# Rayhane-mamah/Tacotron-2

Measured on NVIDIA H100. Metric: wavenet_train_audio_samples_per_sec, higher is better.
Workload: dtype bf16

## Files before the change

### include/t2b200.h

```cpp
#ifndef T2B200_H_
#define T2B200_H_

#include <stdint.h>

#ifdef __cplusplus
extern "C" {
#endif

#define T2B200_ABI_VERSION 2

#define T2_OK 0
#define T2_ERR_INVALID_ARG (-1)
#define T2_ERR_UNSUPPORTED_SHAPE (-2)
#define T2_ERR_CUDA (-3)
#define T2_ERR_NCCL (-4)

const char* t2_last_error(void);
int t2_abi_version(void);
int t2_struct_size(const char* name);
long long t2_launch_count(void);

int t2_dbg_conv_gemm(const void* d_a, int B, int T, int C, int ld, const int* shifts, int nshift,
                     const void* d_w, int N, int BN, const float* d_bias, int relu, void* d_out_bf16,
                     float* d_out_f32, void* stream);
// ... 20 lines not shown
  int cluster_used;
  void* ptr[12];
  float f[6];
  int i[12];
  unsigned long long seed;
} t2_dbg_gemm_t;
int t2_dbg_act_gemm(t2_dbg_gemm_t* call, void* stream);
typedef struct {
  int a_map, a_ch0, a_shift, a_layer;
  int b_map, b_ch0, b_shift, b_layer;
  long long out_off;
  int ldc, m_valid, n_valid;
  float scale;
  int accumulate;
  const float* div;
} t2_dbg_wgrad_tile_t;
int t2_dbg_wgrad_tiles(const t2_dbg_act_t* maps, int nmaps, const t2_dbg_wgrad_tile_t* tiles, int ntiles, float* d_out, int T, int B,
                       void* stream);
int t2_dbg_fx_colsum(const float* d_addends, int nrows, int ncols, float* d_out, void* stream);

typedef struct {
  int kernel;
  void* p[16];
  long long i[16];
  float f[4];
  unsigned long long seed;
  const unsigned long long* step;
} t2_dbg_kernel_t;
#define T2_DBG_TACO_ATT_FWD 1
#define T2_DBG_TACO_BN_FWD 2
// ... 197 lines not shown
```

### tacotron-2_b200/csrc/t2_api.cu

```cuda
#include <stdarg.h>
#include <stdio.h>
#include <stddef.h>
#include <string.h>

#include <vector>

#include "../../include/t2b200.h"
#include "t2_common.cuh"
#include "t2_gemm.h"

#include <atomic>
static thread_local char g_err[512] = "";
static std::atomic<long long> g_launches{0};
void t2_count_launch(int n) { g_launches.fetch_add(n, std::memory_order_relaxed); }
extern "C" long long t2_launch_count(void) { return g_launches.load(std::memory_order_relaxed); }

int t2_set_error(int code, const char* fmt, ...) {
  va_list ap;
  va_start(ap, fmt);
  vsnprintf(g_err, sizeof(g_err), fmt, ap);
  va_end(ap);
  return code;
}

// ... 48 lines not shown
}

#define T2_SAME_FIELD(A, B, f) static_assert(offsetof(A, f) == offsetof(B, f), #A " / " #B ": field " #f)
static_assert(sizeof(t2_dbg_act_t) == sizeof(t2::ActT), "t2_dbg_act_t / ActT");
T2_SAME_FIELD(t2_dbg_act_t, t2::ActT, ptr); T2_SAME_FIELD(t2_dbg_act_t, t2::ActT, C); T2_SAME_FIELD(t2_dbg_act_t, t2::ActT, ld);
static_assert(sizeof(t2_dbg_seg_t) == sizeof(t2::Seg), "t2_dbg_seg_t / Seg");
T2_SAME_FIELD(t2_dbg_seg_t, t2::Seg, map); T2_SAME_FIELD(t2_dbg_seg_t, t2::Seg, nlayers);
static_assert(sizeof(t2_dbg_wgrad_tile_t) == sizeof(t2::WgradTile), "t2_dbg_wgrad_tile_t / WgradTile");
T2_SAME_FIELD(t2_dbg_wgrad_tile_t, t2::WgradTile, a_map); T2_SAME_FIELD(t2_dbg_wgrad_tile_t, t2::WgradTile, a_ch0);
T2_SAME_FIELD(t2_dbg_wgrad_tile_t, t2::WgradTile, a_shift); T2_SAME_FIELD(t2_dbg_wgrad_tile_t, t2::WgradTile, a_layer);
T2_SAME_FIELD(t2_dbg_wgrad_tile_t, t2::WgradTile, b_map); T2_SAME_FIELD(t2_dbg_wgrad_tile_t, t2::WgradTile, b_ch0);
T2_SAME_FIELD(t2_dbg_wgrad_tile_t, t2::WgradTile, b_shift); T2_SAME_FIELD(t2_dbg_wgrad_tile_t, t2::WgradTile, b_layer);
T2_SAME_FIELD(t2_dbg_wgrad_tile_t, t2::WgradTile, out_off); T2_SAME_FIELD(t2_dbg_wgrad_tile_t, t2::WgradTile, ldc);
T2_SAME_FIELD(t2_dbg_wgrad_tile_t, t2::WgradTile, m_valid); T2_SAME_FIELD(t2_dbg_wgrad_tile_t, t2::WgradTile, n_valid);
T2_SAME_FIELD(t2_dbg_wgrad_tile_t, t2::WgradTile, scale); T2_SAME_FIELD(t2_dbg_wgrad_tile_t, t2::WgradTile, accumulate);
T2_SAME_FIELD(t2_dbg_wgrad_tile_t, t2::WgradTile, div);
#undef T2_SAME_FIELD

extern "C" int t2_dbg_act_gemm(t2_dbg_gemm_t* call, void* stream) {
  using namespace t2;
  T2_REQUIRE(call != nullptr, T2_ERR_INVALID_ARG, "null call");
  T2_REQUIRE(call->na >= 1 && call->na <= 4 && call->nseg >= 1 && call->nseg <= kMaxSeg, T2_ERR_INVALID_ARG,
             "bad map/segment count (%d, %d)", call->na, call->nseg);
  ActGemmCall c;
  memset(&c, 0, sizeof(c));
  memcpy(c.a, call->a, sizeof(c.a));
  c.na = call->na;
  memcpy(c.seg, call->seg, sizeof(c.seg));
  c.nseg = call->nseg;
  c.w = call->w; c.wN = call->wN; c.wK = call->wK; c.wL = call->wL; c.w_layer = call->w_layer; c.w_k0 = call->w_k0;
  c.T = call->T; c.B = call->B; c.n_tiles = call->n_tiles; c.ksplit = call->ksplit; c.cluster = call->cluster;
  memcpy(c.epi.ptr, call->ptr, sizeof(c.epi.ptr));
  memcpy(c.epi.f, call->f, sizeof(c.epi.f));
  memcpy(c.epi.i, call->i, sizeof(c.epi.i));
  c.epi.seed = call->seed;
  call->cluster_used = 0;
  return launch_act_gemm(call->epi, call->BN, c, static_cast<cudaStream_t>(stream), &call->cluster_used);
}

extern "C" int t2_dbg_wgrad_tiles(const t2_dbg_act_t* maps, int nmaps, const t2_dbg_wgrad_tile_t* tiles, int ntiles, float* d_out, int T,
                                  int B, void* stream) {
  using namespace t2;
  T2_REQUIRE(maps && tiles && nmaps >= 1 && nmaps <= 6 && ntiles >= 1, T2_ERR_INVALID_ARG, "wgrad_tiles: bad map/tile arguments");
  for (int i = 0; i < ntiles; ++i)
    T2_REQUIRE(tiles[i].a_map >= 0 && tiles[i].a_map < nmaps && tiles[i].b_map >= 0 && tiles[i].b_map < nmaps &&
               tiles[i].m_valid >= 1 && tiles[i].m_valid <= 128 && tiles[i].n_valid >= 1 && tiles[i].n_valid <= 256 &&
               tiles[i].accumulate >= 0 && tiles[i].accumulate <= 2,
               T2_ERR_INVALID_ARG, "wgrad_tiles: bad tile %d", i);
  WgradTile* dt = nullptr;
  cudaStream_t st = static_cast<cudaStream_t>(stream);
  T2_CHECK_CUDA(cudaMallocAsync(&dt, ntiles * sizeof(WgradTile), st));
  const cudaError_t e = cudaMemcpyAsync(dt, tiles, ntiles * sizeof(WgradTile), cudaMemcpyHostToDevice, st);
  int rc = e == cudaSuccess ? launch_wgrad(reinterpret_cast<const ActT*>(maps), nmaps, dt, ntiles, d_out, T, B, st)
                            : t2_set_error(T2_ERR_CUDA, "wgrad_tiles: tile table upload failed: %s", cudaGetErrorString(e));
  cudaStreamSynchronize(st);
  cudaFreeAsync(dt, st);
  return rc;
}

__global__ void fx_colsum_kernel(const float* __restrict__ v, long long n, int ncols, long long* acc) {
  const long long i = blockIdx.x * (long long)blockDim.x + threadIdx.x;
  if (i < n) t2::fx_add(acc + i % ncols, v[i]);
}
extern "C" int t2_dbg_fx_colsum(const float* d_addends, int nrows, int ncols, float* d_out, void* stream) {
  T2_REQUIRE(d_addends && d_out && nrows >= 0 && ncols >= 1, T2_ERR_INVALID_ARG, "fx_colsum: bad arguments");
  cudaStream_t st = static_cast<cudaStream_t>(stream);
  long long* acc = nullptr;
  T2_CHECK_CUDA(cudaMallocAsync(&acc, size_t(ncols) * sizeof(long long), st));
// ... 48 lines not shown
```

### tacotron-2_b200/csrc/t2_gemm.cu

```cuda
#include <stdlib.h>
#include <mutex>

#include "t2_gemm.cuh"
#include "t2_gemm.h"

namespace t2 {

static long long* g_timing_buffer = nullptr;
void set_timing_buffer(long long* p) { g_timing_buffer = p; }

typedef CUresult (*EncodeTiledFn)(CUtensorMap*, CUtensorMapDataType, cuuint32_t, void*, const cuuint64_t*,
                                  const cuuint64_t*, const cuuint32_t*, const cuuint32_t*,
                                  CUtensorMapInterleave, CUtensorMapSwizzle, CUtensorMapL2promotion,
                                  CUtensorMapFloatOOBfill);

static EncodeTiledFn get_encode_fn() {
  static EncodeTiledFn fn = nullptr;
  static std::once_flag once;
  std::call_once(once, [] {
    void* p = nullptr;
    cudaDriverEntryPointQueryResult q;
    if (cudaGetDriverEntryPoint("cuTensorMapEncodeTiled", &p, cudaEnableDefault, &q) == cudaSuccess &&
        q == cudaDriverEntryPointSuccess)
      fn = reinterpret_cast<EncodeTiledFn>(p);
// ... 176 lines not shown
  T2_CASE(EPI_BIAS_ACT, 256)
  T2_CASE(EPI_CE, 256)
  T2_CASE(EPI_SCALE_RELUMASK, 128)
  T2_CASE(EPI_SCALE_RELUMASK, 256)
  T2_CASE(EPI_GATE_BWD, 128)
  T2_CASE(EPI_GATE_BWD, 256)
  T2_CASE(EPI_DX, 128)
  T2_CASE(EPI_DX, 256)
  T2_CASE(EPI_MOL, 32)
  T2_CASE(EPI_LSTM, 32)
  T2_CASE(EPI_TOUT, 32)
#undef T2_CASE
  return t2_set_error(T2_ERR_UNSUPPORTED_SHAPE, "act_gemm: no kernel for epilogue %d with BN=%d", epi, BN);
}

int launch_wgrad(const ActT* maps, int nmaps, const WgradTile* tiles_dev, int ntiles, float* out, int T,
                 int B, cudaStream_t stream) {
  T2_REQUIRE(nmaps >= 1 && nmaps <= 6 && ntiles >= 1, T2_ERR_INVALID_ARG, "wgrad: bad map/tile count");
  WgradArgs g;
  memset(&g, 0, sizeof(g));
  for (int i = 0; i < 6; ++i) {
    int rc = encode_act_map(&g.map[i], maps[i < nmaps ? i : 0], kBK);
    if (rc) return rc;
  }
  g.tiles = tiles_dev;
  g.out = out;
  g.T = T;
  g.B = B;
  static bool configured = false;
  if (!configured) {
    T2_CHECK_CUDA(cudaFuncSetAttribute(wgrad_gemm_kernel, cudaFuncAttributeMaxDynamicSharedMemorySize, kWgSmemBytes));
    configured = true;
  }
  cudaLaunchConfig_t cfg;
  memset(&cfg, 0, sizeof(cfg));
  cfg.gridDim = dim3(ntiles); cfg.blockDim = dim3(kGemmThreads); cfg.dynamicSmemBytes = kWgSmemBytes; cfg.stream = stream;
  cudaLaunchAttribute attr[1];
  attr[0].id = cudaLaunchAttributeProgrammaticStreamSerialization;
  attr[0].val.programmaticStreamSerializationAllowed = 1;
  cfg.attrs = attr; cfg.numAttrs = pdl_enabled() ? 1 : 0;
  T2_CHECK_CUDA(cudaLaunchKernelEx(&cfg, wgrad_gemm_kernel, g));
  t2_count_launch();
  return T2_OK;
}

}
```

### tacotron-2_b200/csrc/t2_gemm.cuh

```cuda
#pragma once
#include "t2_common.cuh"
#include "t2_gemm_types.h"

namespace t2 {

__device__ __forceinline__ void store_bf16x32(__nv_bfloat16* dst, const float (&v)[32]) {
  uint4* d = reinterpret_cast<uint4*>(dst);
#pragma unroll
  for (int q = 0; q < 4; ++q) {
    uint4 u;
    u.x = pack_bf16x2(v[q * 8 + 0], v[q * 8 + 1]);
    u.y = pack_bf16x2(v[q * 8 + 2], v[q * 8 + 3]);
    u.z = pack_bf16x2(v[q * 8 + 4], v[q * 8 + 5]);
    u.w = pack_bf16x2(v[q * 8 + 6], v[q * 8 + 7]);
    d[q] = u;
  }
}
__device__ __forceinline__ void load_bf16x32(const __nv_bfloat16* src, float (&v)[32]) {
  const uint4* s = reinterpret_cast<const uint4*>(src);
#pragma unroll
  for (int q = 0; q < 4; ++q) {
    uint4 u = __ldg(s + q);
    v[q * 8 + 0] = bf16lo(u.x); v[q * 8 + 1] = bf16hi(u.x);
    v[q * 8 + 2] = bf16lo(u.y); v[q * 8 + 3] = bf16hi(u.y);
// ... 984 lines not shown
    asm volatile("bar.sync 6, 512;\n" ::: "memory");
    const int row = q * 32 + lane;
    c.trow = AccRow{acc_s + row * BN, 0, row & 7};
    if (dbg && threadIdx.x == 0) dbg[4] = clock64();
    Epilogue<EPI, BN>::run(g.epi, c);
    if (dbg && threadIdx.x == 0) dbg[5] = clock64();
    tile_store_drain(c);
  }
  __syncthreads();
  if (dbg && threadIdx.x == 0) { dbg[6] = clock64(); dbg[10] = globaltimer_ns(); }
  if (cs > 1) cluster_sync_all();
}

constexpr int kWgBN = 256;
constexpr int kWgStages = 4;
constexpr int kWgStageBytes = 6 * (kBK * 128);
constexpr int kWgSmemBytes = kWgStages * kWgStageBytes + 1024 + 256;
static_assert(kWgSmemBytes <= 232448, "shared memory budget");

template <int N>
__device__ __forceinline__ void wgrad_consume(const WgradArgs& g, const WgradTile& tile, uint8_t* smem, uint64_t* full_bar,
                                              uint64_t* empty_bar, int total_kb) {
  constexpr int kBlk = kBK * 128;
  const int warp = threadIdx.x >> 5, lane = threadIdx.x & 31, wg = warp >> 2;
  float d[N / 2];
#pragma unroll
  for (int i = 0; i < N / 2; ++i) d[i] = 0.f;
  int stage = 0, prev = 0;
  uint32_t phase = 0;
  for (int kb = 0; kb < total_kb; ++kb) {
    mbar_wait(&full_bar[stage], phase);
    __syncwarp();
    const uint32_t sa = smem_u32(smem + stage * kWgStageBytes) + uint32_t(wg * kBlk);
    const uint32_t sb = smem_u32(smem + stage * kWgStageBytes + 2 * kBlk);
    const uint64_t adesc = make_gdesc_sw128(sa, kBlk, 1024);
    const uint64_t bdesc = make_gdesc_sw128(sb, kBlk, 1024);
    wgmma_fence();
    wgmma_fence_regs(d);
#pragma unroll
    for (int k = 0; k < kBK / 16; ++k)
      Wgmma<N, 1, 1>::mma(d, adesc + uint64_t(k * 128), bdesc + uint64_t(k * 128), (kb > 0 || k > 0) ? 1u : 0u);
    wgmma_commit();
    wgmma_fence_regs(d);
    wgmma_wait<1>();
    if (kb > 0 && lane == 0) mbar_arrive(&empty_bar[prev]);
    prev = stage;
    if (++stage == kWgStages) { stage = 0; phase ^= 1; }
  }
  wgmma_wait<0>();
  wgmma_fence_regs(d);
  float sc = tile.scale;
  if (tile.div) sc /= fmaxf(__ldg(tile.div), 1e-20f);
  float* out = g.out + tile.out_off;
  const int m0 = wg * 64 + (warp & 3) * 16 + (lane >> 2);
#pragma unroll
  for (int j = 0; j < N / 8; ++j)
#pragma unroll
    for (int i = 0; i < 2; ++i)
#pragma unroll
      for (int e = 0; e < 2; ++e) {
        const int m = m0 + 8 * i, n = 8 * j + 2 * (lane & 3) + e;
        if (m < tile.m_valid && n < tile.n_valid) {
          float* o = out + size_t(m) * tile.ldc + n;
          const float r = d[4 * j + 2 * i + e] * sc;
          if (tile.accumulate == 2) atomicAdd(o, r);
          else if (tile.accumulate == 1) *o += r;
          else *o = r;
        }
      }
}

__global__ void __launch_bounds__(kGemmThreads, 1) wgrad_gemm_kernel(const __grid_constant__ WgradArgs g) {
  extern __shared__ uint8_t smem_raw[];
  uint8_t* smem = reinterpret_cast<uint8_t*>((reinterpret_cast<uintptr_t>(smem_raw) + 1023) & ~uintptr_t(1023));
  uint64_t* full_bar = reinterpret_cast<uint64_t*>(smem + kWgStages * kWgStageBytes);
  uint64_t* empty_bar = full_bar + kWgStages;
  const int warp = threadIdx.x >> 5;
  const WgradTile tile = g.tiles[blockIdx.x];
  const int kb_per_b = (g.T + kBK - 1) / kBK;
  const int total_kb = kb_per_b * g.B;
  const int nblk = (tile.n_valid + 63) >> 6;

  if (warp == 8 && elect_one()) {
    for (int i = 0; i < kWgStages; ++i) { mbar_init(&full_bar[i], 1); mbar_init(&empty_bar[i], 8); }
    fence_barrier_init();
  }
  __syncthreads();
  pdl_wait();
  pdl_launch_dependents();
  constexpr int kBlk = kBK * 128;

  if (warp == 8) {
    if (elect_one()) {
      int stage = 0; uint32_t phase = 0;
      for (int bb = 0; bb < g.B; ++bb)
        for (int kb = 0; kb < kb_per_b; ++kb) {
          mbar_wait(&empty_bar[stage], phase ^ 1);
          mbar_expect_tx(&full_bar[stage], uint32_t(2 + nblk) * kBlk);
          uint8_t* sa = smem + stage * kWgStageBytes;
          uint8_t* sb = sa + 2 * kBlk;
          const int tpos = kb * kBK;
          tma_load_4d(sa, &g.map[tile.a_map], &full_bar[stage], tile.a_ch0, tpos + tile.a_shift, bb, tile.a_layer);
          tma_load_4d(sa + kBlk, &g.map[tile.a_map], &full_bar[stage], tile.a_ch0 + 64, tpos + tile.a_shift, bb, tile.a_layer);
          for (int i = 0; i < nblk; ++i)
            tma_load_4d(sb + i * kBlk, &g.map[tile.b_map], &full_bar[stage], tile.b_ch0 + 64 * i, tpos + tile.b_shift, bb, tile.b_layer);
          if (++stage == kWgStages) { stage = 0; phase ^= 1; }
        }
    }
  } else {
    switch (nblk) {
      case 1: wgrad_consume<64>(g, tile, smem, full_bar, empty_bar, total_kb); break;
      case 2: wgrad_consume<128>(g, tile, smem, full_bar, empty_bar, total_kb); break;
      case 3: wgrad_consume<192>(g, tile, smem, full_bar, empty_bar, total_kb); break;
      default: wgrad_consume<256>(g, tile, smem, full_bar, empty_bar, total_kb); break;
    }
  }
}

}
```

### tacotron-2_b200/csrc/t2_gemm.h

```cpp
#pragma once
#include <cuda_runtime.h>
#include <string.h>

#include "t2_gemm_types.h"

namespace t2 {

struct ActT {
  const void* ptr;
  int C, T, B, L, ld;
};
inline ActT make_act(const void* p, int C, int T, int B, int L = 1, int ld = -1) {
  ActT a;
  a.ptr = p; a.C = C; a.T = T; a.B = B; a.L = L; a.ld = ld < 0 ? C : ld;
  return a;
}

struct ActGemmCall {
  ActT a[4];
  int na;
  Seg seg[kMaxSeg];
  int nseg;
  const void* w;
  int wN, wK, wL, w_layer, w_k0;
// ... 7 lines not shown
void set_timing_buffer(long long* p);
bool pdl_enabled();
template <typename... KArgs, typename... Args>
inline cudaError_t launch_pdl(void (*kernel)(KArgs...), dim3 grid, dim3 block, size_t smem, cudaStream_t st, Args... args) {
  cudaLaunchConfig_t cfg;
  memset(&cfg, 0, sizeof(cfg));
  cfg.gridDim = grid; cfg.blockDim = block; cfg.dynamicSmemBytes = smem; cfg.stream = st;
  cudaLaunchAttribute attr[1];
  attr[0].id = cudaLaunchAttributeProgrammaticStreamSerialization;
  attr[0].val.programmaticStreamSerializationAllowed = 1;
  cfg.attrs = attr; cfg.numAttrs = pdl_enabled() ? 1 : 0;
  return cudaLaunchKernelEx(&cfg, kernel, KArgs(args)...);
}
int launch_act_gemm(int epi, int BN, const ActGemmCall& c, cudaStream_t stream, int* cluster_used = nullptr);
int launch_wgrad(const ActT* maps, int nmaps, const WgradTile* tiles_dev, int ntiles, float* out,
                 int T, int B, cudaStream_t stream);

}
```

### tacotron-2_b200/csrc/t2_gemm_types.h

```cpp
#pragma once
#include <cuda.h>
#include <stdint.h>

namespace t2 {

constexpr int kBM = 128;
constexpr int kBK = 64;
constexpr int kMaxSeg = 16;
constexpr int kGemmThreads = 288;
constexpr int kDbgSlots = 16;

struct Seg {
  int map;
  int shift;
  int k0;
  int nkb;
  int layer0;
  int nlayers;
};

struct EpiArgs {
  void* ptr[12];
  float f[6];
  int i[12];
// ... 25 lines not shown
  EPI_DX = 7,
  EPI_LSTM = 8,
  EPI_TOUT = 9,
};


struct WgradTile {
  int a_map, a_ch0, a_shift, a_layer;
  int b_map, b_ch0, b_shift, b_layer;
  long long out_off;
  int ldc;
  int m_valid, n_valid;
  float scale;
  int accumulate;
  const float* div;
};
struct WgradArgs {
  CUtensorMap map[6];
  const WgradTile* tiles;
  float* out;
  int T, B;
};

}
```

### tacotron-2_b200/csrc/t2_wavenet.cu

```cuda
#include <stdlib.h>
#include <math.h>
#include <stdio.h>
#include <string.h>

#include <algorithm>
#include <string>
#include <vector>

#include "../../include/t2b200.h"
#include "t2_common.cuh"
#include "t2_gemm.h"

namespace t2 {
namespace {

typedef __nv_bfloat16 bf16;

struct PackJob {
  long long src_off;
  int K, N;
  long long dst_off;
  int dst_ld;
  int transpose;
  int col0;
// ... 256 lines not shown

  lo.tiles_main.clear();
  auto wt = [&](std::vector<WgradTile>& v, int am, int ach, int ash, int al, int bm, int bch, int bl, long long off,
                int ldc, int mv, int nv, float scale, const float* div) {
    WgradTile t; memset(&t, 0, sizeof(t));
    t.a_map = am; t.a_ch0 = ach; t.a_shift = ash; t.a_layer = al; t.b_map = bm; t.b_ch0 = bch; t.b_shift = 0; t.b_layer = bl;
    t.out_off = off; t.ldc = ldc; t.m_valid = mv; t.n_valid = nv; t.scale = scale; t.accumulate = 0; t.div = div;
    v.push_back(t);
  };
  const int WN = 256;
  auto nmin = [&](int rem) { return rem < WN ? rem : WN; };
  lo.tile_start.assign(lo.L + 1, 0);
  for (int l = 0; l < lo.L; ++l) {
    const int d = lo.dil(l);
    lo.tile_start[l] = int(lo.tiles_main.size());
    for (int j = 0; j < 3; ++j)
      for (int m0 = 0; m0 < lo.R; m0 += 128)
        for (int n0 = 0; n0 < lo.G; n0 += WN)
          wt(lo.tiles_main, 0, m0, -(2 - j) * d, l, 1, n0, l, lo.p_dil_k[l] + (long long)j * lo.R * lo.G + (long long)m0 * lo.G + n0,
             lo.G, 128, nmin(lo.G - n0), 1.f, nullptr);
    if (lo.C > 0)
      for (int n0 = 0; n0 < lo.G; n0 += WN)
        wt(lo.tiles_main, 2, 0, 0, 0, 1, n0, l, lo.p_c_k[l] + n0, lo.G, lo.C, nmin(lo.G - n0), 1.f, nullptr);
    for (int m0 = 0; m0 < lo.Gh; m0 += 128) {
      if (l < lo.L - 1)
        for (int n0 = 0; n0 < lo.R; n0 += WN)
          wt(lo.tiles_main, 3, m0, 0, l, 4, n0, l + 1, lo.p_o_k[l] + (long long)m0 * lo.R + n0, lo.R, 128, nmin(lo.R - n0), lo.res_scale, nullptr);
      for (int n0 = 0; n0 < lo.S; n0 += WN)
        wt(lo.tiles_main, 3, m0, 0, l, 5, n0, 0, lo.p_s_k[l] + (long long)m0 * lo.S + n0, lo.S, 128, nmin(lo.S - n0), lo.skip_scale[l], nullptr);
    }
  }
  lo.tiles_head.clear();
  for (int m0 = 0; m0 < lo.S; m0 += 128) {
    for (int n0 = 0; n0 < lo.S; n0 += WN)
      wt(lo.tiles_head, 0, m0, 0, 0, 1, n0, 0, lo.p_f1_k + (long long)m0 * lo.S + n0, lo.S, 128, nmin(lo.S - n0), 1.f, nullptr);
// ... 1108 lines not shown
  int rc = build_layout(cfg, lo);
  if (rc) return rc;
  cudaStream_t st = static_cast<cudaStream_t>(stream);
  T2_REQUIRE(!lo.split, T2_ERR_INVALID_ARG, "split_bf16 (fp32-class) mode has no backward pass");
  T2_REQUIRE(n_groups >= 1 && n_groups <= lo.L && (phase == -1 || phase == 100 || (phase >= 0 && phase <= n_groups)), T2_ERR_INVALID_ARG,
             "backward_phased: bad phase %d / n_groups %d", phase, n_groups);
  if (phase >= 1 && phase <= n_groups) {
    uint8_t* ws = static_cast<uint8_t*>(d_workspace);
    const int g = phase - 1;
    const int l0 = int((long long)lo.L * g / n_groups), l1 = int((long long)lo.L * (g + 1) / n_groups);
    const int t0 = lo.tile_start[l0], t1 = lo.tile_start[l1];
    ActT maps[6] = {make_act(ws + lo.w_xd, lo.R, lo.T, lo.B, lo.L), make_act(ws + lo.w_dg, lo.G, lo.T, lo.B, lo.L),
                    make_act(ws + lo.w_cup, lo.C > 0 ? lo.C : 8, lo.T, lo.B, 1),
                    make_act(ws + lo.w_z, lo.Gh, lo.T, lo.B, lo.L), make_act(ws + lo.w_dxin, lo.R, lo.T, lo.B, lo.L),
                    make_act(ws + lo.w_dskip, lo.S, lo.T, lo.B, 1)};
    return launch_wgrad(maps, 6, reinterpret_cast<const WgradTile*>(ws + lo.w_tiles_main) + t0, t1 - t0, d_grads, lo.T, lo.B, st);
  }
  if (phase == 100) {
    SideStream* side = side_stream();
    if (side) {
      T2_CHECK_CUDA(cudaEventRecord(side->join, side->s));
      T2_CHECK_CUDA(cudaStreamWaitEvent(st, side->join, 0));
    }
    return launch_fx_finalize(reinterpret_cast<const long long*>(static_cast<uint8_t*>(d_workspace) + lo.w_gfx), d_grads, lo.n_params, st);
  }
  uint8_t* ws = static_cast<uint8_t*>(d_workspace);
  const uint8_t* pk = static_cast<const uint8_t*>(d_packed);
  const long long BT = (long long)lo.B * lo.T;
  float* scalars = reinterpret_cast<float*>(ws + lo.w_scalars);
  const float p = cfg->dropout;
  T2_CHECK_CUDA(cudaMemsetAsync(d_grads, 0, lo.n_params * sizeof(float), st));
// ... 71 lines not shown
    a.offs = reinterpret_cast<const long long*>(ws + lo.w_tables);
    a.p_k = lo.p_g_k[0]; a.p_b = lo.p_g_b[0]; a.p_stride = lo.layer_stride; a.p_emb = lo.p_emb;
    a.L = lo.L; a.B = lo.B; a.G = lo.G; a.Gi = lo.Gi; a.NS = lo.NS;
    gin_wgrad_kernel<<<grid1d((long long)lo.L * lo.G), 256, 0, st>>>(a); t2_count_launch();
    gin_demb_kernel<<<dim3(lo.NS, lo.Gi), kGinThreads, 0, st>>>(a); t2_count_launch();
    T2_CHECK_CUDA(cudaGetLastError());
  }
  if (side) {
    T2_CHECK_CUDA(cudaEventRecord(side->fork2, st));
    T2_CHECK_CUDA(cudaStreamWaitEvent(side->s, side->fork2, 0));
  }
  if (phase == -1) {
    ActT maps[6] = {make_act(ws + lo.w_xd, lo.R, lo.T, lo.B, lo.L), a_dg,
                    make_act(ws + lo.w_cup, lo.C > 0 ? lo.C : 8, lo.T, lo.B, 1),
                    make_act(ws + lo.w_z, lo.Gh, lo.T, lo.B, lo.L), a_dxin, a_dskip};
    rc = launch_wgrad(maps, 6, reinterpret_cast<const WgradTile*>(ws + lo.w_tiles_main), lo.n_tiles_main, d_grads, lo.T, lo.B, st);
    if (rc) return rc;
  }
  first_conv_bwd_kernel<<<dim3((unsigned)((BT + 63) / 64)), lo.R, 0, sb>>>(d_x, lo.scalar_in ? 1 : 0, dxin, gfx + lo.p_in_k, BT, lo.R); t2_count_launch();
  T2_CHECK_CUDA(cudaGetLastError());
  if (lo.C > 0 && !cfg->c_pre_upsampled) {
    float* dcup = reinterpret_cast<float*>(ws + lo.w_dcup);
    ActGemmCall g;
    memset(&g, 0, sizeof(g));
    g.a[0] = a_dg; g.na = 1;
    g.seg[0] = Seg{0, 0, 0, lo.G / kBK, 0, lo.L}; g.nseg = 1;
    g.w = pk + lo.k_WcT; g.wN = lo.C; g.wK = lo.L * lo.G; g.wL = 1;
    g.T = lo.T; g.B = lo.B; g.n_tiles = 1;
    g.epi.ptr[0] = nullptr; g.epi.ptr[1] = nullptr; g.epi.ptr[2] = dcup;
    g.epi.i[0] = lo.C; g.epi.i[1] = 0; g.epi.i[2] = lo.C;
    rc = launch_act_gemm(EPI_BIAS_ACT, 128, g, sb);
// ... 45 lines not shown

extern "C" int t2_wn_workspace_tensor(const t2_wn_config_t* cfg, void* d_workspace, const char* name, void** ptr,
                                      long long* count, int* elem_bytes) {
  Layout lo;
  int rc = build_layout(cfg, lo);
  if (rc) return rc;
  uint8_t* ws = static_cast<uint8_t*>(d_workspace);
  const long long BT = (long long)lo.B * lo.T;
  struct E { const char* n; long long off; long long cnt; int eb; };
  const E table[] = {
      {"c_up", lo.w_cup, BT * lo.C, 2},       {"x", lo.w_x, lo.L * BT * lo.R, 2},    {"xd", lo.w_xd, lo.L * BT * lo.R, 2},
      {"ta", lo.w_ta, lo.L * BT * lo.Gh, 2},  {"sb", lo.w_sb, lo.L * BT * lo.Gh, 2}, {"z", lo.w_z, lo.L * BT * lo.Gh, 2},
      {"h1", lo.w_h1, BT * lo.S, 2},          {"h2", lo.w_h2, BT * lo.S, 2},         {"dlog", lo.w_dlog, BT * lo.ldo, 2},
      {"dh2", lo.w_dh2, BT * lo.S, 2},        {"dskip", lo.w_dskip, BT * lo.S, 2},   {"dxin", lo.w_dxin, lo.L * BT * lo.R, 2},
      {"dg", lo.w_dg, lo.L * BT * lo.G, 2},   {"dc_up", lo.w_dcup, BT * lo.C, 4},    {"scalars", lo.w_scalars, 16, 4},
  };
  for (const E& e : table)
    if (strcmp(e.n, name) == 0) {
      *ptr = ws + e.off; *count = e.cnt; *elem_bytes = e.eb;
      return T2_OK;
    }
  return t2_set_error(T2_ERR_INVALID_ARG, "unknown workspace tensor '%s'", name);
}

extern "C" int t2_dbg_wn_kernel(const t2_dbg_kernel_t* call, void* stream) {
  T2_REQUIRE(call != nullptr, T2_ERR_INVALID_ARG, "dbg_wn_kernel: null call");
  cudaStream_t st = static_cast<cudaStream_t>(stream);
  void* const* p = call->p;
  const long long* i = call->i;
  const long long B = i[0], C = i[1], W = i[2], s = i[3], type = i[4], act = i[5];
// ... 25 lines not shown
    }
    case T2_DBG_WN_UP_BWD_INPUT:
      T2_REQUIRE(p[0] && p[1] && p[2] && p[3], T2_ERR_INVALID_ARG, "dbg_wn_kernel UP_BWD_INPUT: null pointer argument");
      return launch_upsample_bwd_input(static_cast<const float*>(p[0]), static_cast<const float*>(p[1]), static_cast<const float*>(p[2]),
                                       static_cast<float*>(p[3]), b, c, w, sc, ty, ac, alpha, st);
    default:
      return t2_set_error(T2_ERR_INVALID_ARG, "dbg_wn_kernel: unknown kernel id %d", call->kernel);
  }
}

extern "C" int t2_wn_time_kernel(const t2_wn_config_t* cfg, const float* d_params, const void* d_packed, void* d_workspace,
                                 int which, int layer, int reps, float* ms_per_launch, void* stream) {
  Layout lo;
  int rc = build_layout(cfg, lo);
  if (rc) return rc;
  T2_REQUIRE(layer >= 0 && layer < lo.L && reps >= 1 && ms_per_launch && which >= 0 && which <= 4, T2_ERR_INVALID_ARG,
             "time_kernel: bad arguments");
  T2_REQUIRE(which != 1 || layer + 1 < lo.L, T2_ERR_INVALID_ARG, "the last layer has no out GEMM");
  cudaStream_t st = static_cast<cudaStream_t>(stream);
  uint8_t* ws = static_cast<uint8_t*>(d_workspace);
  const uint8_t* pk = static_cast<const uint8_t*>(d_packed);
  ActGemmCall g;
  int epi, bn;
  if (which == 0 || which == 4) { g = make_gate_call(lo, ws, pk, layer, which == 0); epi = EPI_GATE; bn = 256; }
  else if (which == 1) { g = make_out_call(lo, ws, pk, d_params, layer, cfg->dropout, 1, nullptr); epi = EPI_RES; bn = lo.R; }
  else if (which == 2) { g = make_dz_call(lo, ws, pk, layer, nullptr); epi = EPI_GATE_BWD; bn = lo.Gh >= 256 ? 256 : 128; }
  else { g = make_dx_call(lo, ws, pk, layer, cfg->dropout, 1, nullptr, nullptr); epi = EPI_DX; bn = lo.R; }
  T2_CHECK_CUDA(cudaStreamSynchronize(st));
  cudaStream_t ps;
  T2_CHECK_CUDA(cudaStreamCreateWithFlags(&ps, cudaStreamNonBlocking));
  cudaEvent_t e0, e1;
  T2_CHECK_CUDA(cudaEventCreate(&e0));
  T2_CHECK_CUDA(cudaEventCreate(&e1));
  rc = launch_act_gemm(epi, bn, g, ps);
  if (rc) return rc;
  T2_CHECK_CUDA(cudaStreamSynchronize(ps));
  cudaGraph_t graph;
  cudaGraphExec_t exec;
  T2_CHECK_CUDA(cudaStreamBeginCapture(ps, cudaStreamCaptureModeThreadLocal));
  for (int i = 0; i < reps && rc == 0; ++i) rc = launch_act_gemm(epi, bn, g, ps);
  cudaError_t ce = cudaStreamEndCapture(ps, &graph);
  if (rc) return rc;
  T2_CHECK_CUDA(ce);
  T2_CHECK_CUDA(cudaGraphInstantiate(&exec, graph, 0));
  T2_CHECK_CUDA(cudaGraphLaunch(exec, ps));
  T2_CHECK_CUDA(cudaEventRecord(e0, ps));
  T2_CHECK_CUDA(cudaGraphLaunch(exec, ps));
  T2_CHECK_CUDA(cudaEventRecord(e1, ps));
  T2_CHECK_CUDA(cudaEventSynchronize(e1));
  float ms = 0.f;
  T2_CHECK_CUDA(cudaEventElapsedTime(&ms, e0, e1));
  *ms_per_launch = ms / reps;
  cudaGraphExecDestroy(exec);
  cudaGraphDestroy(graph);
  cudaEventDestroy(e0);
  cudaEventDestroy(e1);
  cudaStreamDestroy(ps);
  return T2_OK;
}

#include <cooperative_groups.h>
namespace cg = cooperative_groups;

namespace t2 {
namespace {

constexpr int kArThreads = 512;
__device__ long long* g_ar_dbg = nullptr;
#define AR_STAMP(i) do { if (g_ar_dbg && blockIdx.x == 0 && threadIdx.x == 0 && t == 64 && l == 7) g_ar_dbg[i] = clock64(); } while (0)
constexpr int kArMaxItems = 4;

struct ArLayout {
// ... 628 lines not shown
```

### tacotron-2_b200/lib.py

```python
import ctypes
import os

_HERE = os.path.dirname(os.path.abspath(__file__))
LIB_PATH = os.environ.get("T2_LIB") or os.path.join(_HERE, "libt2b200.so")
_lib = None


class T2Error(RuntimeError):
    pass


def load():
    global _lib
    if _lib is None:
        if not os.path.exists(LIB_PATH):
            raise T2Error("libt2b200.so is not built: run `python __graft_entry__.py build` "
                          "(there is no CPU fallback for the CUDA hot path)")
        _lib = ctypes.CDLL(LIB_PATH)
        _lib.t2_last_error.restype = ctypes.c_char_p
        _lib.t2_launch_count.restype = ctypes.c_longlong
    return _lib


def check(rc):
# ... 24 lines not shown

class DbgGemm(ctypes.Structure):
    _fields_ = [("a", DbgAct * 4), ("na", ctypes.c_int),
                ("seg", DbgSeg * 16), ("nseg", ctypes.c_int),
                ("w", ctypes.c_void_p), ("wN", ctypes.c_int), ("wK", ctypes.c_int), ("wL", ctypes.c_int),
                ("w_layer", ctypes.c_int), ("w_k0", ctypes.c_int),
                ("T", ctypes.c_int), ("B", ctypes.c_int), ("n_tiles", ctypes.c_int), ("ksplit", ctypes.c_int),
                ("epi", ctypes.c_int), ("BN", ctypes.c_int), ("cluster", ctypes.c_int), ("cluster_used", ctypes.c_int),
                ("ptr", ctypes.c_void_p * 12), ("f", ctypes.c_float * 6), ("i", ctypes.c_int * 12), ("seed", ctypes.c_ulonglong)]


class DbgWgradTile(ctypes.Structure):
    _fields_ = [("a_map", ctypes.c_int), ("a_ch0", ctypes.c_int), ("a_shift", ctypes.c_int), ("a_layer", ctypes.c_int),
                ("b_map", ctypes.c_int), ("b_ch0", ctypes.c_int), ("b_shift", ctypes.c_int), ("b_layer", ctypes.c_int),
                ("out_off", ctypes.c_longlong), ("ldc", ctypes.c_int), ("m_valid", ctypes.c_int), ("n_valid", ctypes.c_int),
                ("scale", ctypes.c_float), ("accumulate", ctypes.c_int), ("div", ctypes.c_void_p)]


class DbgKernel(ctypes.Structure):
    _fields_ = [("kernel", ctypes.c_int), ("p", ctypes.c_void_p * 16), ("i", ctypes.c_longlong * 16), ("f", ctypes.c_float * 4),
                ("seed", ctypes.c_ulonglong), ("step", ctypes.c_void_p)]
```

Baseline: 3.629 million.

## Fuse three dilated-conv tap weight-gradient tiles into one three-slab wgrad tile

The dilated-conv weight-gradient tiles used to issue one 128-row tile per kernel tap (3 taps), each reloading the same B operand (dg). They are replaced by 64-row tiles that load three shifted A slabs per stage, so the three taps share one B load across three warpgroups. A new NS=3 kernel variant drops the dedicated producer warp: the last consumer to release a stage, found with a shared-memory atomic counter, issues the next TMA loads. This trades fewer B loads for a different synchronisation scheme and twice as many smaller M tiles. It also adds a timing hook for the wgrad kernel.

```diff
diff --git a/include/t2b200.h b/include/t2b200.h
--- a/include/t2b200.h
+++ b/include/t2b200.h
@@ -58,6 +58,8 @@
   float scale;
   int accumulate;
   const float* div;
+  int slabs, slab_shift_step;
+  long long slab_out_step;
 } t2_dbg_wgrad_tile_t;
 int t2_dbg_wgrad_tiles(const t2_dbg_act_t* maps, int nmaps, const t2_dbg_wgrad_tile_t* tiles, int ntiles, float* d_out, int T, int B,
                        void* stream);
diff --git a/tacotron-2_b200/csrc/t2_api.cu b/tacotron-2_b200/csrc/t2_api.cu
--- a/tacotron-2_b200/csrc/t2_api.cu
+++ b/tacotron-2_b200/csrc/t2_api.cu
@@ -86,7 +86,8 @@
 T2_SAME_FIELD(t2_dbg_wgrad_tile_t, t2::WgradTile, out_off); T2_SAME_FIELD(t2_dbg_wgrad_tile_t, t2::WgradTile, ldc);
 T2_SAME_FIELD(t2_dbg_wgrad_tile_t, t2::WgradTile, m_valid); T2_SAME_FIELD(t2_dbg_wgrad_tile_t, t2::WgradTile, n_valid);
 T2_SAME_FIELD(t2_dbg_wgrad_tile_t, t2::WgradTile, scale); T2_SAME_FIELD(t2_dbg_wgrad_tile_t, t2::WgradTile, accumulate);
-T2_SAME_FIELD(t2_dbg_wgrad_tile_t, t2::WgradTile, div);
+T2_SAME_FIELD(t2_dbg_wgrad_tile_t, t2::WgradTile, div); T2_SAME_FIELD(t2_dbg_wgrad_tile_t, t2::WgradTile, slabs);
+T2_SAME_FIELD(t2_dbg_wgrad_tile_t, t2::WgradTile, slab_shift_step); T2_SAME_FIELD(t2_dbg_wgrad_tile_t, t2::WgradTile, slab_out_step);
 #undef T2_SAME_FIELD
 
 extern "C" int t2_dbg_act_gemm(t2_dbg_gemm_t* call, void* stream) {
@@ -114,16 +115,20 @@
                                   int B, void* stream) {
   using namespace t2;
   T2_REQUIRE(maps && tiles && nmaps >= 1 && nmaps <= 6 && ntiles >= 1, T2_ERR_INVALID_ARG, "wgrad_tiles: bad map/tile arguments");
-  for (int i = 0; i < ntiles; ++i)
-    T2_REQUIRE(tiles[i].a_map >= 0 && tiles[i].a_map < nmaps && tiles[i].b_map >= 0 && tiles[i].b_map < nmaps &&
-               tiles[i].m_valid >= 1 && tiles[i].m_valid <= 128 && tiles[i].n_valid >= 1 && tiles[i].n_valid <= 256 &&
-               tiles[i].accumulate >= 0 && tiles[i].accumulate <= 2,
+  int slabs = 2;
+  for (int i = 0; i < ntiles; ++i) {
+    const t2_dbg_wgrad_tile_t& t = tiles[i];
+    T2_REQUIRE(t.a_map >= 0 && t.a_map < nmaps && t.b_map >= 0 && t.b_map < nmaps && t.m_valid >= 1 &&
+               t.m_valid <= (t.slabs ? 64 : 128) && t.n_valid >= 1 && t.n_valid <= 256 && t.accumulate >= 0 && t.accumulate <= 2 &&
+               (t.slabs == 3 || (t.slabs == 0 && t.slab_shift_step == 0 && t.slab_out_step == 0)),
                T2_ERR_INVALID_ARG, "wgrad_tiles: bad tile %d", i);
+    if (t.slabs) slabs = 3;
+  }
   WgradTile* dt = nullptr;
   cudaStream_t st = static_cast<cudaStream_t>(stream);
   T2_CHECK_CUDA(cudaMallocAsync(&dt, ntiles * sizeof(WgradTile), st));
   const cudaError_t e = cudaMemcpyAsync(dt, tiles, ntiles * sizeof(WgradTile), cudaMemcpyHostToDevice, st);
-  int rc = e == cudaSuccess ? launch_wgrad(reinterpret_cast<const ActT*>(maps), nmaps, dt, ntiles, d_out, T, B, st)
+  int rc = e == cudaSuccess ? launch_wgrad(reinterpret_cast<const ActT*>(maps), nmaps, dt, ntiles, d_out, T, B, st, slabs)
                             : t2_set_error(T2_ERR_CUDA, "wgrad_tiles: tile table upload failed: %s", cudaGetErrorString(e));
   cudaStreamSynchronize(st);
   cudaFreeAsync(dt, st);
diff --git a/tacotron-2_b200/csrc/t2_gemm.cu b/tacotron-2_b200/csrc/t2_gemm.cu
--- a/tacotron-2_b200/csrc/t2_gemm.cu
+++ b/tacotron-2_b200/csrc/t2_gemm.cu
@@ -214,9 +214,29 @@
   return t2_set_error(T2_ERR_UNSUPPORTED_SHAPE, "act_gemm: no kernel for epilogue %d with BN=%d", epi, BN);
 }
 
+template <int NS>
+static int launch_wgrad_ns(const WgradArgs& g, int ntiles, cudaStream_t stream) {
+  static bool configured = false;
+  if (!configured) {
+    T2_CHECK_CUDA(cudaFuncSetAttribute(wgrad_gemm_kernel<NS>, cudaFuncAttributeMaxDynamicSharedMemorySize, WgCfg<NS>::kSmemBytes));
+    configured = true;
+  }
+  cudaLaunchConfig_t cfg;
+  memset(&cfg, 0, sizeof(cfg));
+  cfg.gridDim = dim3(ntiles); cfg.blockDim = dim3(WgCfg<NS>::kThreads); cfg.dynamicSmemBytes = WgCfg<NS>::kSmemBytes; cfg.stream = stream;
+  cudaLaunchAttribute attr[1];
+  attr[0].id = cudaLaunchAttributeProgrammaticStreamSerialization;
+  attr[0].val.programmaticStreamSerializationAllowed = 1;
+  cfg.attrs = attr; cfg.numAttrs = pdl_enabled() ? 1 : 0;
+  T2_CHECK_CUDA(cudaLaunchKernelEx(&cfg, wgrad_gemm_kernel<NS>, g));
+  t2_count_launch();
+  return T2_OK;
+}
+
 int launch_wgrad(const ActT* maps, int nmaps, const WgradTile* tiles_dev, int ntiles, float* out, int T,
-                 int B, cudaStream_t stream) {
+                 int B, cudaStream_t stream, int slabs) {
   T2_REQUIRE(nmaps >= 1 && nmaps <= 6 && ntiles >= 1, T2_ERR_INVALID_ARG, "wgrad: bad map/tile count");
+  T2_REQUIRE(slabs == 2 || slabs == 3, T2_ERR_INVALID_ARG, "wgrad: slabs must be 2 or 3 (got %d)", slabs);
   WgradArgs g;
   memset(&g, 0, sizeof(g));
   for (int i = 0; i < 6; ++i) {
@@ -227,21 +247,7 @@
   g.out = out;
   g.T = T;
   g.B = B;
-  static bool configured = false;
-  if (!configured) {
-    T2_CHECK_CUDA(cudaFuncSetAttribute(wgrad_gemm_kernel, cudaFuncAttributeMaxDynamicSharedMemorySize, kWgSmemBytes));
-    configured = true;
-  }
-  cudaLaunchConfig_t cfg;
-  memset(&cfg, 0, sizeof(cfg));
-  cfg.gridDim = dim3(ntiles); cfg.blockDim = dim3(kGemmThreads); cfg.dynamicSmemBytes = kWgSmemBytes; cfg.stream = stream;
-  cudaLaunchAttribute attr[1];
-  attr[0].id = cudaLaunchAttributeProgrammaticStreamSerialization;
-  attr[0].val.programmaticStreamSerializationAllowed = 1;
-  cfg.attrs = attr; cfg.numAttrs = pdl_enabled() ? 1 : 0;
-  T2_CHECK_CUDA(cudaLaunchKernelEx(&cfg, wgrad_gemm_kernel, g));
-  t2_count_launch();
-  return T2_OK;
-}
-
-}
+  return slabs == 3 ? launch_wgrad_ns<3>(g, ntiles, stream) : launch_wgrad_ns<2>(g, ntiles, stream);
+}
+
+}
diff --git a/tacotron-2_b200/csrc/t2_gemm.cuh b/tacotron-2_b200/csrc/t2_gemm.cuh
--- a/tacotron-2_b200/csrc/t2_gemm.cuh
+++ b/tacotron-2_b200/csrc/t2_gemm.cuh
@@ -1022,13 +1022,35 @@
 
 constexpr int kWgBN = 256;
 constexpr int kWgStages = 4;
-constexpr int kWgStageBytes = 6 * (kBK * 128);
-constexpr int kWgSmemBytes = kWgStages * kWgStageBytes + 1024 + 256;
-static_assert(kWgSmemBytes <= 232448, "shared memory budget");
-
-template <int N>
+template <int NS>
+struct WgCfg {
+  static constexpr int kThreads = NS == 2 ? 2 * 128 + 32 : NS * 128;
+  static constexpr int kStageBytes = (NS + 4) * (kBK * 128);
+  static constexpr int kSmemBytes = kWgStages * kStageBytes + 1024 + 256;
+  static_assert(kSmemBytes <= 232448, "shared memory budget");
+};
+static_assert(WgCfg<2>::kThreads == kGemmThreads, "two-slab wgrad block");
+
+template <int NS>
+__device__ __forceinline__ void wgrad_issue(const WgradArgs& g, const WgradTile& tile, uint8_t* smem, uint64_t* full_bar, int kbg,
+                                            int stage, int nslab, int nblk, int kb_per_b) {
+  constexpr int kBlk = kBK * 128;
+  const int bb = kbg / kb_per_b, tpos = (kbg - bb * kb_per_b) * kBK;
+  mbar_expect_tx(&full_bar[stage], uint32_t(nslab + nblk) * kBlk);
+  uint8_t* sa = smem + stage * WgCfg<NS>::kStageBytes;
+  uint8_t* sb = sa + NS * kBlk;
+  for (int s = 0; s < nslab; ++s) {
+    const int ch = tile.slabs ? tile.a_ch0 : tile.a_ch0 + 64 * s;
+    const int sh = tile.slabs ? tile.a_shift + s * tile.slab_shift_step : tile.a_shift;
+    tma_load_4d(sa + s * kBlk, &g.map[tile.a_map], &full_bar[stage], ch, tpos + sh, bb, tile.a_layer);
+  }
+  for (int i = 0; i < nblk; ++i)
+    tma_load_4d(sb + i * kBlk, &g.map[tile.b_map], &full_bar[stage], tile.b_ch0 + 64 * i, tpos + tile.b_shift, bb, tile.b_layer);
+}
+
+template <int N, int NS>
 __device__ __forceinline__ void wgrad_consume(const WgradArgs& g, const WgradTile& tile, uint8_t* smem, uint64_t* full_bar,
-                                              uint64_t* empty_bar, int total_kb) {
+                                              uint64_t* empty_bar, int total_kb, int nslab = 2, int kb_per_b = 0) {
   constexpr int kBlk = kBK * 128;
   const int warp = threadIdx.x >> 5, lane = threadIdx.x & 31, wg = warp >> 2;
   float d[N / 2];
@@ -1039,8 +1061,8 @@
   for (int kb = 0; kb < total_kb; ++kb) {
     mbar_wait(&full_bar[stage], phase);
     __syncwarp();
-    const uint32_t sa = smem_u32(smem + stage * kWgStageBytes) + uint32_t(wg * kBlk);
-    const uint32_t sb = smem_u32(smem + stage * kWgStageBytes + 2 * kBlk);
+    const uint32_t sa = smem_u32(smem + stage * WgCfg<NS>::kStageBytes) + uint32_t(wg * kBlk);
+    const uint32_t sb = smem_u32(smem + stage * WgCfg<NS>::kStageBytes + NS * kBlk);
     const uint64_t adesc = make_gdesc_sw128(sa, kBlk, 1024);
     const uint64_t bdesc = make_gdesc_sw128(sb, kBlk, 1024);
     wgmma_fence();
@@ -1051,7 +1073,16 @@
     wgmma_commit();
     wgmma_fence_regs(d);
     wgmma_wait<1>();
-    if (kb > 0 && lane == 0) mbar_arrive(&empty_bar[prev]);
+    if constexpr (NS == 2) {
+      if (kb > 0 && lane == 0) mbar_arrive(&empty_bar[prev]);
+    } else if (kb > 0 && lane == 0) {
+      int* released = reinterpret_cast<int*>(empty_bar);
+      if (atomicAdd(&released[prev], 1) == 4 * nslab - 1) {
+        released[prev] = 0;
+        if (kb - 1 + kWgStages < total_kb)
+          wgrad_issue<NS>(g, tile, smem, full_bar, kb - 1 + kWgStages, prev, nslab, (tile.n_valid + 63) >> 6, kb_per_b);
+      }
+    }
     prev = stage;
     if (++stage == kWgStages) { stage = 0; phase ^= 1; }
   }
@@ -1060,7 +1091,13 @@
   float sc = tile.scale;
   if (tile.div) sc /= fmaxf(__ldg(tile.div), 1e-20f);
   float* out = g.out + tile.out_off;
-  const int m0 = wg * 64 + (warp & 3) * 16 + (lane >> 2);
+  int m0 = wg * 64 + (warp & 3) * 16 + (lane >> 2);
+  if constexpr (NS > 2) {
+    if (tile.slabs) {
+      out += wg * tile.slab_out_step;
+      m0 -= wg * 64;
+    }
+  }
 #pragma unroll
   for (int j = 0; j < N / 8; ++j)
 #pragma unroll
@@ -1078,10 +1115,12 @@
       }
 }
 
-__global__ void __launch_bounds__(kGemmThreads, 1) wgrad_gemm_kernel(const __grid_constant__ WgradArgs g) {
+template <int NS>
+__global__ void __launch_bounds__(WgCfg<NS>::kThreads, 1) wgrad_gemm_kernel(const __grid_constant__ WgradArgs g) {
+  using Cfg = WgCfg<NS>;
   extern __shared__ uint8_t smem_raw[];
   uint8_t* smem = reinterpret_cast<uint8_t*>((reinterpret_cast<uintptr_t>(smem_raw) + 1023) & ~uintptr_t(1023));
-  uint64_t* full_bar = reinterpret_cast<uint64_t*>(smem + kWgStages * kWgStageBytes);
+  uint64_t* full_bar = reinterpret_cast<uint64_t*>(smem + kWgStages * Cfg::kStageBytes);
   uint64_t* empty_bar = full_bar + kWgStages;
   const int warp = threadIdx.x >> 5;
   const WgradTile tile = g.tiles[blockIdx.x];
@@ -1089,40 +1128,60 @@
   const int total_kb = kb_per_b * g.B;
   const int nblk = (tile.n_valid + 63) >> 6;
 
-  if (warp == 8 && elect_one()) {
-    for (int i = 0; i < kWgStages; ++i) { mbar_init(&full_bar[i], 1); mbar_init(&empty_bar[i], 8); }
-    fence_barrier_init();
-  }
-  __syncthreads();
-  pdl_wait();
-  pdl_launch_dependents();
-  constexpr int kBlk = kBK * 128;
-
-  if (warp == 8) {
-    if (elect_one()) {
-      int stage = 0; uint32_t phase = 0;
-      for (int bb = 0; bb < g.B; ++bb)
-        for (int kb = 0; kb < kb_per_b; ++kb) {
-          mbar_wait(&empty_bar[stage], phase ^ 1);
-          mbar_expect_tx(&full_bar[stage], uint32_t(2 + nblk) * kBlk);
-          uint8_t* sa = smem + stage * kWgStageBytes;
-          uint8_t* sb = sa + 2 * kBlk;
-          const int tpos = kb * kBK;
-          tma_load_4d(sa, &g.map[tile.a_map], &full_bar[stage], tile.a_ch0, tpos + tile.a_shift, bb, tile.a_layer);
-          tma_load_4d(sa + kBlk, &g.map[tile.a_map], &full_bar[stage], tile.a_ch0 + 64, tpos + tile.a_shift, bb, tile.a_layer);
-          for (int i = 0; i < nblk; ++i)
-            tma_load_4d(sb + i * kBlk, &g.map[tile.b_map], &full_bar[stage], tile.b_ch0 + 64 * i, tpos + tile.b_shift, bb, tile.b_layer);
-          if (++stage == kWgStages) { stage = 0; phase ^= 1; }
-        }
+  if constexpr (NS == 2) {
+    if (warp == 8 && elect_one()) {
+      for (int i = 0; i < kWgStages; ++i) { mbar_init(&full_bar[i], 1); mbar_init(&empty_bar[i], 8); }
+      fence_barrier_init();
+    }
+    __syncthreads();
+    pdl_wait();
+    pdl_launch_dependents();
+    constexpr int kBlk = kBK * 128;
+
+    if (warp == 8) {
+      if (elect_one()) {
+        int stage = 0; uint32_t phase = 0;
+        for (int bb = 0; bb < g.B; ++bb)
+          for (int kb = 0; kb < kb_per_b; ++kb) {
+            mbar_wait(&empty_bar[stage], phase ^ 1);
+            mbar_expect_tx(&full_bar[stage], uint32_t(2 + nblk) * kBlk);
+            uint8_t* sa = smem + stage * Cfg::kStageBytes;
+            uint8_t* sb = sa + 2 * kBlk;
+            const int tpos = kb * kBK;
+            tma_load_4d(sa, &g.map[tile.a_map], &full_bar[stage], tile.a_ch0, tpos + tile.a_shift, bb, tile.a_layer);
+            tma_load_4d(sa + kBlk, &g.map[tile.a_map], &full_bar[stage], tile.a_ch0 + 64, tpos + tile.a_shift, bb, tile.a_layer);
+            for (int i = 0; i < nblk; ++i)
+              tma_load_4d(sb + i * kBlk, &g.map[tile.b_map], &full_bar[stage], tile.b_ch0 + 64 * i, tpos + tile.b_shift, bb, tile.b_layer);
+            if (++stage == kWgStages) { stage = 0; phase ^= 1; }
+          }
+      }
+    } else {
+      switch (nblk) {
+        case 1: wgrad_consume<64, NS>(g, tile, smem, full_bar, empty_bar, total_kb); break;
+        case 2: wgrad_consume<128, NS>(g, tile, smem, full_bar, empty_bar, total_kb); break;
+        case 3: wgrad_consume<192, NS>(g, tile, smem, full_bar, empty_bar, total_kb); break;
+        default: wgrad_consume<256, NS>(g, tile, smem, full_bar, empty_bar, total_kb); break;
+      }
     }
   } else {
+    const int nslab = tile.slabs ? NS : 2;
+    if (threadIdx.x == 0) {
+      for (int i = 0; i < kWgStages; ++i) { mbar_init(&full_bar[i], 1); reinterpret_cast<int*>(empty_bar)[i] = 0; }
+      fence_barrier_init();
+    }
+    __syncthreads();
+    pdl_wait();
+    pdl_launch_dependents();
+    if (threadIdx.x == 0)
+      for (int kb = 0; kb < kWgStages && kb < total_kb; ++kb) wgrad_issue<NS>(g, tile, smem, full_bar, kb, kb, nslab, nblk, kb_per_b);
+    if ((warp >> 2) >= nslab) return;
     switch (nblk) {
-      case 1: wgrad_consume<64>(g, tile, smem, full_bar, empty_bar, total_kb); break;
-      case 2: wgrad_consume<128>(g, tile, smem, full_bar, empty_bar, total_kb); break;
-      case 3: wgrad_consume<192>(g, tile, smem, full_bar, empty_bar, total_kb); break;
-      default: wgrad_consume<256>(g, tile, smem, full_bar, empty_bar, total_kb); break;
-    }
-  }
-}
-
-}
+      case 1: wgrad_consume<64, NS>(g, tile, smem, full_bar, empty_bar, total_kb, nslab, kb_per_b); break;
+      case 2: wgrad_consume<128, NS>(g, tile, smem, full_bar, empty_bar, total_kb, nslab, kb_per_b); break;
+      case 3: wgrad_consume<192, NS>(g, tile, smem, full_bar, empty_bar, total_kb, nslab, kb_per_b); break;
+      default: wgrad_consume<256, NS>(g, tile, smem, full_bar, empty_bar, total_kb, nslab, kb_per_b); break;
+    }
+  }
+}
+
+}
diff --git a/tacotron-2_b200/csrc/t2_gemm.h b/tacotron-2_b200/csrc/t2_gemm.h
--- a/tacotron-2_b200/csrc/t2_gemm.h
+++ b/tacotron-2_b200/csrc/t2_gemm.h
@@ -45,6 +45,6 @@
 }
 int launch_act_gemm(int epi, int BN, const ActGemmCall& c, cudaStream_t stream, int* cluster_used = nullptr);
 int launch_wgrad(const ActT* maps, int nmaps, const WgradTile* tiles_dev, int ntiles, float* out,
-                 int T, int B, cudaStream_t stream);
+                 int T, int B, cudaStream_t stream, int slabs = 2);
 
 }
diff --git a/tacotron-2_b200/csrc/t2_gemm_types.h b/tacotron-2_b200/csrc/t2_gemm_types.h
--- a/tacotron-2_b200/csrc/t2_gemm_types.h
+++ b/tacotron-2_b200/csrc/t2_gemm_types.h
@@ -63,6 +63,9 @@
   float scale;
   int accumulate;
   const float* div;
+  int slabs;
+  int slab_shift_step;
+  long long slab_out_step;
 };
 struct WgradArgs {
   CUtensorMap map[6];
diff --git a/tacotron-2_b200/csrc/t2_wavenet.cu b/tacotron-2_b200/csrc/t2_wavenet.cu
--- a/tacotron-2_b200/csrc/t2_wavenet.cu
+++ b/tacotron-2_b200/csrc/t2_wavenet.cu
@@ -294,11 +294,12 @@
   for (int l = 0; l < lo.L; ++l) {
     const int d = lo.dil(l);
     lo.tile_start[l] = int(lo.tiles_main.size());
-    for (int j = 0; j < 3; ++j)
-      for (int m0 = 0; m0 < lo.R; m0 += 128)
-        for (int n0 = 0; n0 < lo.G; n0 += WN)
-          wt(lo.tiles_main, 0, m0, -(2 - j) * d, l, 1, n0, l, lo.p_dil_k[l] + (long long)j * lo.R * lo.G + (long long)m0 * lo.G + n0,
-             lo.G, 128, nmin(lo.G - n0), 1.f, nullptr);
+    for (int m0 = 0; m0 < lo.R; m0 += 64)
+      for (int n0 = 0; n0 < lo.G; n0 += WN) {
+        wt(lo.tiles_main, 0, m0, -2 * d, l, 1, n0, l, lo.p_dil_k[l] + (long long)m0 * lo.G + n0, lo.G, 64, nmin(lo.G - n0), 1.f, nullptr);
+        WgradTile& t = lo.tiles_main.back();
+        t.slabs = 3; t.slab_shift_step = d; t.slab_out_step = (long long)lo.R * lo.G;
+      }
     if (lo.C > 0)
       for (int n0 = 0; n0 < lo.G; n0 += WN)
         wt(lo.tiles_main, 2, 0, 0, 0, 1, n0, l, lo.p_c_k[l] + n0, lo.G, lo.C, nmin(lo.G - n0), 1.f, nullptr);
@@ -1437,7 +1438,7 @@
                     make_act(ws + lo.w_cup, lo.C > 0 ? lo.C : 8, lo.T, lo.B, 1),
                     make_act(ws + lo.w_z, lo.Gh, lo.T, lo.B, lo.L), make_act(ws + lo.w_dxin, lo.R, lo.T, lo.B, lo.L),
                     make_act(ws + lo.w_dskip, lo.S, lo.T, lo.B, 1)};
-    return launch_wgrad(maps, 6, reinterpret_cast<const WgradTile*>(ws + lo.w_tiles_main) + t0, t1 - t0, d_grads, lo.T, lo.B, st);
+    return launch_wgrad(maps, 6, reinterpret_cast<const WgradTile*>(ws + lo.w_tiles_main) + t0, t1 - t0, d_grads, lo.T, lo.B, st, 3);
   }
   if (phase == 100) {
     SideStream* side = side_stream();
@@ -1539,7 +1540,7 @@
     ActT maps[6] = {make_act(ws + lo.w_xd, lo.R, lo.T, lo.B, lo.L), a_dg,
                     make_act(ws + lo.w_cup, lo.C > 0 ? lo.C : 8, lo.T, lo.B, 1),
                     make_act(ws + lo.w_z, lo.Gh, lo.T, lo.B, lo.L), a_dxin, a_dskip};
-    rc = launch_wgrad(maps, 6, reinterpret_cast<const WgradTile*>(ws + lo.w_tiles_main), lo.n_tiles_main, d_grads, lo.T, lo.B, st);
+    rc = launch_wgrad(maps, 6, reinterpret_cast<const WgradTile*>(ws + lo.w_tiles_main), lo.n_tiles_main, d_grads, lo.T, lo.B, st, 3);
     if (rc) return rc;
   }
   first_conv_bwd_kernel<<<dim3((unsigned)((BT + 63) / 64)), lo.R, 0, sb>>>(d_x, lo.scalar_in ? 1 : 0, dxin, gfx + lo.p_in_k, BT, lo.R); t2_count_launch();
@@ -1615,6 +1616,7 @@
       {"h1", lo.w_h1, BT * lo.S, 2},          {"h2", lo.w_h2, BT * lo.S, 2},         {"dlog", lo.w_dlog, BT * lo.ldo, 2},
       {"dh2", lo.w_dh2, BT * lo.S, 2},        {"dskip", lo.w_dskip, BT * lo.S, 2},   {"dxin", lo.w_dxin, lo.L * BT * lo.R, 2},
       {"dg", lo.w_dg, lo.L * BT * lo.G, 2},   {"dc_up", lo.w_dcup, BT * lo.C, 4},    {"scalars", lo.w_scalars, 16, 4},
+      {"wgrad_tiles", lo.w_tiles_main, lo.n_tiles_main, int(sizeof(WgradTile))},
   };
   for (const E& e : table)
     if (strcmp(e.n, name) == 0) {
@@ -1670,31 +1672,42 @@
   Layout lo;
   int rc = build_layout(cfg, lo);
   if (rc) return rc;
-  T2_REQUIRE(layer >= 0 && layer < lo.L && reps >= 1 && ms_per_launch && which >= 0 && which <= 4, T2_ERR_INVALID_ARG,
+  T2_REQUIRE(layer >= 0 && layer < lo.L && reps >= 1 && ms_per_launch && which >= 0 && which <= 5, T2_ERR_INVALID_ARG,
              "time_kernel: bad arguments");
   T2_REQUIRE(which != 1 || layer + 1 < lo.L, T2_ERR_INVALID_ARG, "the last layer has no out GEMM");
   cudaStream_t st = static_cast<cudaStream_t>(stream);
   uint8_t* ws = static_cast<uint8_t*>(d_workspace);
   const uint8_t* pk = static_cast<const uint8_t*>(d_packed);
   ActGemmCall g;
-  int epi, bn;
+  int epi = 0, bn = 0;
   if (which == 0 || which == 4) { g = make_gate_call(lo, ws, pk, layer, which == 0); epi = EPI_GATE; bn = 256; }
   else if (which == 1) { g = make_out_call(lo, ws, pk, d_params, layer, cfg->dropout, 1, nullptr); epi = EPI_RES; bn = lo.R; }
   else if (which == 2) { g = make_dz_call(lo, ws, pk, layer, nullptr); epi = EPI_GATE_BWD; bn = lo.Gh >= 256 ? 256 : 128; }
-  else { g = make_dx_call(lo, ws, pk, layer, cfg->dropout, 1, nullptr, nullptr); epi = EPI_DX; bn = lo.R; }
+  else if (which == 3) { g = make_dx_call(lo, ws, pk, layer, cfg->dropout, 1, nullptr, nullptr); epi = EPI_DX; bn = lo.R; }
+  const ActT wmaps[6] = {make_act(ws + lo.w_xd, lo.R, lo.T, lo.B, lo.L), make_act(ws + lo.w_dg, lo.G, lo.T, lo.B, lo.L),
+                         make_act(ws + lo.w_cup, lo.C > 0 ? lo.C : 8, lo.T, lo.B, 1),
+                         make_act(ws + lo.w_z, lo.Gh, lo.T, lo.B, lo.L), make_act(ws + lo.w_dxin, lo.R, lo.T, lo.B, lo.L),
+                         make_act(ws + lo.w_dskip, lo.S, lo.T, lo.B, 1)};
+  float* wout = nullptr;
+  if (which == 5) T2_CHECK_CUDA(cudaMalloc(&wout, lo.n_params * sizeof(float)));
+  auto launch = [&](cudaStream_t s) {
+    return which == 5 ? launch_wgrad(wmaps, 6, reinterpret_cast<const WgradTile*>(ws + lo.w_tiles_main), lo.n_tiles_main, wout, lo.T,
+                                     lo.B, s, 3)
+                      : launch_act_gemm(epi, bn, g, s);
+  };
   T2_CHECK_CUDA(cudaStreamSynchronize(st));
   cudaStream_t ps;
   T2_CHECK_CUDA(cudaStreamCreateWithFlags(&ps, cudaStreamNonBlocking));
   cudaEvent_t e0, e1;
   T2_CHECK_CUDA(cudaEventCreate(&e0));
   T2_CHECK_CUDA(cudaEventCreate(&e1));
-  rc = launch_act_gemm(epi, bn, g, ps);
+  rc = launch(ps);
   if (rc) return rc;
   T2_CHECK_CUDA(cudaStreamSynchronize(ps));
   cudaGraph_t graph;
   cudaGraphExec_t exec;
   T2_CHECK_CUDA(cudaStreamBeginCapture(ps, cudaStreamCaptureModeThreadLocal));
-  for (int i = 0; i < reps && rc == 0; ++i) rc = launch_act_gemm(epi, bn, g, ps);
+  for (int i = 0; i < reps && rc == 0; ++i) rc = launch(ps);
   cudaError_t ce = cudaStreamEndCapture(ps, &graph);
   if (rc) return rc;
   T2_CHECK_CUDA(ce);
@@ -1712,6 +1725,7 @@
   cudaEventDestroy(e0);
   cudaEventDestroy(e1);
   cudaStreamDestroy(ps);
+  if (wout) T2_CHECK_CUDA(cudaFree(wout));
   return T2_OK;
 }
 
diff --git a/tacotron-2_b200/lib.py b/tacotron-2_b200/lib.py
--- a/tacotron-2_b200/lib.py
+++ b/tacotron-2_b200/lib.py
@@ -62,7 +62,8 @@
     _fields_ = [("a_map", ctypes.c_int), ("a_ch0", ctypes.c_int), ("a_shift", ctypes.c_int), ("a_layer", ctypes.c_int),
                 ("b_map", ctypes.c_int), ("b_ch0", ctypes.c_int), ("b_shift", ctypes.c_int), ("b_layer", ctypes.c_int),
                 ("out_off", ctypes.c_longlong), ("ldc", ctypes.c_int), ("m_valid", ctypes.c_int), ("n_valid", ctypes.c_int),
-                ("scale", ctypes.c_float), ("accumulate", ctypes.c_int), ("div", ctypes.c_void_p)]
+                ("scale", ctypes.c_float), ("accumulate", ctypes.c_int), ("div", ctypes.c_void_p),
+                ("slabs", ctypes.c_int), ("slab_shift_step", ctypes.c_int), ("slab_out_step", ctypes.c_longlong)]
 
 
 class DbgKernel(ctypes.Structure):
```

Result: no change. 3.651 million, median of 6 (+0.6%).
